# DiWu9/Union-Thesis-SLAM

Hardware: AMD Instinct MI355X
Metric: depth frames/sec (640x480 into 512^3 @ 2 cm dense TSDF; hash alongside) (higher is better)
Workload: dtype f64

## Files before the change

union-thesis-slam_amd/csrc/tsdf_common.hip:

```cpp
#include <unistd.h>

#include <algorithm>
#include <atomic>
#include <chrono>
#include <cmath>
#include <condition_variable>
#include <cstring>
#include <mutex>
#include <thread>
#include <vector>

#include "tsdf_host.h"

namespace tsdf {

static thread_local std::string g_err;

int set_error(int code, const char* fmt, ...) {
    char buf[1024];
    va_list ap;
    va_start(ap, fmt);
    vsnprintf(buf, sizeof(buf), fmt, ap);
    va_end(ap);
    g_err = buf;
// ... 404 lines not shown
        if (c0 < (size_t)n) {
            TSDF_HIP(hipMemcpyAsync((char*)st_depth[slot] + dbytes * c0, (const char*)hst_depth[slot] + dbytes * c0,
                                    dbytes * (n - c0), hipMemcpyHostToDevice, cstream));
            TSDF_HIP(hipMemcpyAsync((char*)st_color[slot] + cbytes * c0, (const char*)hst_color[slot] + cbytes * c0,
                                    cbytes * (n - c0), hipMemcpyHostToDevice, cstream));
        }
        TSDF_HIP(hipEventRecord(ev_copied[slot], cstream));
        TSDF_HIP(hipStreamWaitEvent(stream, ev_copied[slot], 0));
        d = (const char*)st_depth[slot];
        c = (const char*)st_color[slot];
    }
    const bool mask = (flags & TSDF_DEPTH_INVALID_65535) && dk == TSDF_DEPTH_U16_MM;
    if (mask && (dmask_px < npx || !dmask_set[n_sets - 1])) {
        TSDF_TRY(sync_all());
        for (int k = 0; k < kSets; ++k) {
            if (dmask_set[k]) TSDF_HIP(hipFree(dmask_set[k]));
            dmask_set[k] = nullptr;
        }
        for (int k = 0; k < n_sets; ++k)
            TSDF_HIP(hipMalloc(&dmask_set[k], sizeof(unsigned short) * npx * batch));
        dmask_px = npx;
    }
    use_set(cur_set);
    bt->n = n;
    const bool tex = texel_now && dk == TSDF_DEPTH_U16_MM && ck == TSDF_COLOR_RGB8;
    bt->texel = tex ? 1 : 0;
    for (int i = 0; i < n; ++i) {
        Frame* fr = &bt->f[i];
        const double* T = Tinv + 16 * (size_t)(first + i);
        for (int r = 0; r < 12; ++r) fr->T[r] = T[r];
        fr->fx = (double)(float)K[0];
        fr->fy = (double)(float)K[4];
        fr->cx = (double)(float)K[2];
        fr->cy = (double)(float)K[5];
        for (int j = 0; j < 4; ++j) {
            fr->Tf[j] = T[j] * fr->fx;
            fr->Tf[4 + j] = T[4 + j] * fr->fy;
        }
        {
            double wmax[3];
            for (int a = 0; a < 3; ++a) {
                const long long gmax = (a == 0 ? (long long)vol.off[0] + col_gx(vol, vol.nb[0] - 1) + kBrickEdge
                                               : (long long)vol.off[a] + vol.dims[a]);
                wmax[a] = fabs((double)vol.origin[a]) + vol.vs * (double)gmax + 1.0;
            }
            const PixelFixed pf = pixel_fixed(T, fr->fx, fr->fy, fr->cx, fr->cy, W, H, wmax);
            fr->Cx = pf.Cx;
            fr->Cy = pf.Cy;
            fr->mm = pf.mm;
            fr->whm1 = pf.whm1;
            fr->wmul = pf.wmul;
            fr->zmin_hi = pf.zmin_hi;
        }
        fr->ow = ow ? ow[first + i] : ow_default;
        fr->ow32 = (float)fr->ow;
        fr->H = H;
        fr->W = W;
        fr->depth_src = d + dbytes * i;
        fr->depth_mask = mask ? dmask + npx * i : nullptr;
        fr->depth = mask ? (const void*)fr->depth_mask : fr->depth_src;
        fr->color = c + cbytes * i;
        const bool direct = ck == TSDF_COLOR_RGB8 && rgb_direct &&
                            (!(flags & TSDF_DEVICE_PTRS) || (call_color_end && (const char*)fr->color + cbytes < call_color_end));
        if (tex) fr->rgbx = rgbx + 2 * npx * i;
        else fr->rgbx = direct ? nullptr : rgbx + npx * i;
        fr->pyr = pyr + (size_t)lay.total * i;

        frustum_planes(fr, T, W, H);
    }
    for (int L = 0; L <= kPyrLevels; ++L) {
        bt->pg.off[L] = lay.off[L];
        bt->pg.w[L] = lay.w[L];
        bt->pg.h[L] = lay.h[L];
    }
    return TSDF_OK;
}

int Base::stage_alloc(size_t dbytes, size_t cbytes) {
    if (st_depth_bytes >= dbytes * batch && st_color_bytes >= cbytes * batch) return TSDF_OK;
    TSDF_TRY(sync_all());
    for (int k = 0; k < kSlots; ++k) {
        if (st_depth[k]) TSDF_HIP(hipFree(st_depth[k]));
        if (st_color[k]) TSDF_HIP(hipFree(st_color[k]));
        if (hst_depth[k]) TSDF_HIP(hipHostFree(hst_depth[k]));
        if (hst_color[k]) TSDF_HIP(hipHostFree(hst_color[k]));
        st_depth[k] = st_color[k] = hst_depth[k] = hst_color[k] = nullptr;
    }
    st_depth_bytes = st_color_bytes = 0;
    for (int k = 0; k < kSlots; ++k) {
        TSDF_HIP(hipMalloc(&st_depth[k], dbytes * batch));
        TSDF_HIP(hipMalloc(&st_color[k], cbytes * batch + 64));
        TSDF_HIP(hipHostMalloc(&hst_depth[k], dbytes * batch, hipHostMallocDefault));
        TSDF_HIP(hipHostMalloc(&hst_color[k], cbytes * batch, hipHostMallocDefault));
    }
    st_depth_bytes = dbytes * batch;
    st_color_bytes = cbytes * batch;
    return TSDF_OK;
}

bool Base::defer_same(int dk, int ck, int H, int W, const double* K) const {
    return dfr.dk_in == dk && dfr.ck == ck && dfr.H == H && dfr.W == W && std::memcmp(dfr.K, K, sizeof(dfr.K)) == 0;
}

int Base::defer_push(const void* depth, int dk, const void* color, int ck, int H, int W,
                     const double* K, const double* T, double ow) {
    const size_t cbytes = frame_bytes_color(ck, H, W), npx = (size_t)H * W;
// ... 260 lines not shown
```

union-thesis-slam_amd/csrc/tsdf_device.h:

```cpp
#pragma once
#include <hip/hip_runtime.h>
#include <stdint.h>
#include <type_traits>

#include "tsdf_pixel.h"

namespace tsdf {

constexpr int kBrickEdge = 8;
constexpr int kBrickVox = 512;
constexpr int kWG = 256;
constexpr int kPyrLevels = 6;
constexpr int kStatSpread = 64;
constexpr unsigned long long kEmpty = ~0ull;
constexpr unsigned long long kTomb = ~0ull - 1ull;

enum Stat { ST_VOXELS = 0, ST_VISITED, ST_TOUCHED, ST_ALLOC, ST_PROBE, ST_LOOKUPS, ST_OVERFLOW,
            ST_PROBE_MAX, ST_BAD_ENTRY, ST_UNIQUE, kNStat };

struct Vol {
    int dims[3];
    int off[3];
    int xstride;
    int xodd;
    int sb[3];
    int nb[3];
    int shard, n_shards;
    int canon;
    float origin[3];
    double vs, trunc;
    double rtrunc;
    const double* rcp;
};

__host__ __device__ inline int col_gx(const Vol& v, int c) {
    return (c >> 1) * 2 * v.xstride + (c & 1) * v.xodd;
}

struct Frame {
    double T[12];
    double fx, fy, cx, cy;
    double ow;
    double Tf[8];
    double Cx, Cy;
    unsigned mm, whm1, wmul;
    int zmin_hi;
    float ow32;
    int H, W;
    const void* depth;
    const void* depth_src;
    unsigned short* depth_mask;
    const void* color;
    const unsigned* rgbx;
    const float* pyr;
    float planes[5][4];
    double eye[3];
};

struct PyrGeo {
    int off[kPyrLevels + 1];
    int w[kPyrLevels + 1];
    int h[kPyrLevels + 1];
};

#ifndef TSDF_MAX_BATCH
#define TSDF_MAX_BATCH 32
#endif
constexpr int kMaxBatch = TSDF_MAX_BATCH;
static_assert(kMaxBatch == 8 || kMaxBatch == 16 || kMaxBatch == 32, "frames per batch: 8, 16 or 32");
#ifndef TSDF_FULL_BATCH
#define TSDF_FULL_BATCH TSDF_MAX_BATCH
#endif
constexpr int kFullBatch = TSDF_FULL_BATCH < kMaxBatch ? TSDF_FULL_BATCH : kMaxBatch;
constexpr int kDoneWord = kMaxBatch + 8, kDoneWordC = kMaxBatch + 9, kCursorWord = kMaxBatch + 10;
constexpr int kCountWords = kMaxBatch + 16;
constexpr int kRcpTab = 4096;
constexpr int kRcpBig = 65536;

__device__ inline bool small_int(float w) {
    return w >= 0.0f && w < (float)(kRcpTab - kMaxBatch - 1) && w == truncf(w);
}
__device__ inline bool table_int(float w) {
    return w >= 0.0f && w < (float)(kRcpBig - kMaxBatch - 1) && w == truncf(w);
}
__device__ inline bool canon_color(float c) {
    return c >= 0.0f && c < 16777216.0f && c == truncf(c);
}
struct Batch {
    Frame f[kMaxBatch];
    PyrGeo pg;
    int n;
    int texel;
};

typedef unsigned long long ListEntry;

struct Pool {
    float* tsdf;
    float* weight;
// ... 20 lines not shown
struct Table {
    unsigned long long* keys;
    int* vals;
    unsigned long long* occ;
    int* free_list;
    ListEntry* overflow;
    PoolState* st;
    PoolReport* rb;
    long long capacity;
    long long shard_cap;
    long long max_blocks;
    const int* owned;
    int n_owned;
    int* ins_list;
    long long ins_cap;
    int overflow_cap;
    int int_bits;
};

template <bool POW2 = false>
__host__ __device__ inline long long ref_hash(long long x, long long y, long long z, long long n,
                                              int int_bits) {
    const unsigned long long P1 = 73856093ull, P2 = 19349669ull, P3 = 83492791ull;
    long long h;
    if (int_bits == 32) {
        const int a = (int)(unsigned)((unsigned long long)x * P1);
        const int b = (int)(unsigned)((unsigned long long)y * P2);
        const int c = (int)(unsigned)((unsigned long long)z * P3);
        h = (long long)(a ^ b ^ c);
    } else {
        h = (long long)(((unsigned long long)x * P1) ^ ((unsigned long long)y * P2) ^
                        ((unsigned long long)z * P3));
    }
    if (POW2 || (n & (n - 1)) == 0) return h & (n - 1);
    long long m = h % n;
    return m < 0 ? m + n : m;
}

template <bool POW2 = false>
__host__ __device__ inline int shard_of(long long home, int n_shards, long long cap) {
    if (POW2 || (cap & (cap - 1)) == 0) return (int)((home * n_shards) >> (63 - __builtin_clzll((unsigned long long)cap)));
    return (int)((home * n_shards) / cap);
}

__host__ __device__ inline unsigned long long pack_key(int bx, int by, int bz) {
    return (unsigned long long)bx | ((unsigned long long)by << 21) | ((unsigned long long)bz << 42);
}

__device__ inline int lane_id() { return threadIdx.x & 63; }

__device__ unsigned long long fcmp64_mask(double a, double b, int pred) __asm("llvm.amdgcn.fcmp.i64.f64");
__device__ unsigned long long fcmp32_mask(float a, float b, int pred) __asm("llvm.amdgcn.fcmp.i64.f32");
__device__ unsigned long long icmp32_mask(unsigned a, unsigned b, int pred) __asm("llvm.amdgcn.icmp.i64.i32");
constexpr int kCmpOGT = 2, kCmpOGE = 3, kCmpOLT = 4, kCmpUNE = 14, kCmpEQ = 32, kCmpNE = 33, kCmpULT = 36, kCmpSGT = 38;
__device__ inline bool lane_in(unsigned long long m) { return __builtin_amdgcn_inverse_ballot_w64(m); }
__device__ inline void sel_in_place(float& x, float y, unsigned long long m) {
    asm("v_cndmask_b32 %0, %0, %1, %2" : "+v"(x) : "v"(y), "s"(m));
}

template <typename T>
__device__ inline T coh_load(T* p) {
    return __hip_atomic_load(p, __ATOMIC_RELAXED, __HIP_MEMORY_SCOPE_AGENT);
}
template <typename T>
__device__ inline void coh_store(T* p, T v) {
    __hip_atomic_store(p, v, __ATOMIC_RELAXED, __HIP_MEMORY_SCOPE_AGENT);
}

__device__ inline int hash_find(const Table& t, int bx, int by, int bz, long long n_blocks) {
    const unsigned long long key = pack_key(bx, by, bz);
    long long s = ref_hash(bx, by, bz, t.capacity, t.int_bits);
    for (long long n = 0; n < t.capacity; ++n) {
        const unsigned long long k = coh_load(&t.keys[s]);
        if (k == key) {
            const int blk = coh_load(&t.vals[s]);
            return blk >= 0 && blk < n_blocks ? blk : -1;
        }
        if (k == kEmpty) return -1;
        if (++s == t.capacity) s = 0;
    }
    return -1;
}

__device__ inline double vox_world(float origin, double vs, int g) {
    return (double)(float)((double)origin + vs * (double)g);
}

struct BrickBox {
    double p0[3];
    float ext[3];
    float ctr[3];
    float rad;
};

__device__ inline BrickBox brick_box(const Vol& v, const double* eye, int bx, int by, int bz, int nx = 1,
                                     int ny = 1, int nz = 1) {
    const int bb[3] = {bx, by, bz}, nn[3] = {nx, ny, nz};
    BrickBox r;
#pragma unroll
    for (int a = 0; a < 3; ++a) {
        const int lo = bb[a] * kBrickEdge;
        const int hi = min(lo + nn[a] * kBrickEdge - 1, v.dims[a] - 1);
        const int glo = (a == 0) ? col_gx(v, bb[0]) : lo;
        const int ghi = (a == 0) ? col_gx(v, hi >> 3) + (hi & 7) : hi;
        r.p0[a] = (double)v.origin[a] + v.vs * (double)(glo + v.off[a]);
        r.ext[a] = (float)(v.vs * (double)(ghi - glo));
        r.ctr[a] = (float)(r.p0[a] + 0.5 * v.vs * (double)(ghi - glo) - eye[a]);
// ... 119 lines not shown
            if (ok == 2) {
                slot_out = target;
                probe = scanned + ((target - pos + t.capacity) % t.capacity);
                return coh_load(&t.vals[target]);
            }
            scanned += (target - pos + t.capacity) % t.capacity + 1;
            pos = target + 1;
            if (pos >= t.capacity) pos -= t.capacity;
            tomb = -1;
            continue;
        }
        pos += 64;
        if (pos >= t.capacity) pos -= t.capacity;
        scanned += 64;
    }
    return -1;
}


__device__ unsigned short buf_ld_u16(__amdgpu_buffer_rsrc_t r, int vindex, int voffset, int soffset,
                                     int aux) __asm("llvm.amdgcn.struct.ptr.buffer.load.i16");
__device__ unsigned buf_ld_u32(__amdgpu_buffer_rsrc_t r, int vindex, int voffset, int soffset,
                               int aux) __asm("llvm.amdgcn.struct.ptr.buffer.load.i32");
__device__ double buf_ld_f64(__amdgpu_buffer_rsrc_t r, int vindex, int voffset, int soffset,
                             int aux) __asm("llvm.amdgcn.struct.ptr.buffer.load.f64");
constexpr int kBufDword3 = 0x00020000;
typedef unsigned u32x2 __attribute__((ext_vector_type(2)));
__device__ u32x2 buf_ld_v2u32(__amdgpu_buffer_rsrc_t r, int vindex, int voffset, int soffset,
                              int aux) __asm("llvm.amdgcn.struct.ptr.buffer.load.v2i32");
struct FrameBufs {
    __amdgpu_buffer_rsrc_t depth, color;
};
template <int DK, int CK>
__device__ inline FrameBufs frame_bufs(const Frame& fr) {
    const int n = fr.W * fr.H;
    FrameBufs b;
    if (DK == 2) {
        static_assert(DK != 2 || CK == 0, "texels: RGB8 colour");
        b.depth = b.color = __builtin_amdgcn_make_buffer_rsrc((void*)fr.rgbx, 8, n, kBufDword3);
        return b;
    }
    b.depth = __builtin_amdgcn_make_buffer_rsrc((void*)fr.depth, DK == 0 ? 2 : 8, n, kBufDword3);
    if (CK == 0 && !fr.rgbx) b.color = __builtin_amdgcn_make_buffer_rsrc((void*)fr.color, 3, n, kBufDword3);
    else b.color = __builtin_amdgcn_make_buffer_rsrc((void*)(CK == 0 ? (const void*)fr.rgbx : fr.color), 4, n, kBufDword3);
    return b;
}
template <int DK>
__device__ inline unsigned depth_raw(const FrameBufs& fb, unsigned p) {
    return DK == 0 ? (unsigned)buf_ld_u16(fb.depth, (int)p, 0, 0, 0) : 0u;
}
template <int DK>
__device__ inline double depth_m(const FrameBufs& fb, unsigned p, unsigned raw) {
    if (DK != 1) {
        const double m = DK == 2 ? (double)(int)raw : (double)raw;
        return fma(m, 0.001, m * -2.0858186326137145e-20);
    }
    return buf_ld_f64(fb.depth, (int)p, 0, 0, 0);
}

__device__ inline double div_rn(double a, double b, double y) {
    const double q0 = a * y;
    const double r = fma(-q0, b, a);
    return fma(r, y, q0);
}

__device__ inline float div_rn32(float a, float b, float y) {
    const float q0 = a * y;
    const float r = fmaf(-q0, b, a);
    return fmaf(r, y, q0);
}

typedef float f2 __attribute__((ext_vector_type(2)));
__device__ inline f2 pk_fma(f2 a, f2 b, f2 c) { return __builtin_elementwise_fma(a, b, c); }
__device__ inline f2 rint2(f2 a) { return f2{rintf(a.x), rintf(a.y)}; }
__device__ inline f2 div_rn32x2(f2 a, f2 b, f2 y) {
    const f2 q0 = a * y;
    const f2 r = pk_fma(-q0, b, a);
    return pk_fma(r, y, q0);
}


__device__ inline int cvt_i32_sat(double x) {
    int r;
    asm("v_cvt_i32_f64 %0, %1" : "=v"(r) : "v"(x));
    return r;
}

typedef unsigned short u16x2 __attribute__((ext_vector_type(2)));
__device__ inline unsigned pk_min_u16(unsigned a, unsigned b) {
    return __builtin_bit_cast(unsigned, __builtin_elementwise_min(__builtin_bit_cast(u16x2, a), __builtin_bit_cast(u16x2, b)));
}
__device__ inline unsigned dot2_u16(unsigned a, unsigned b) {
    return __builtin_amdgcn_udot2(__builtin_bit_cast(u16x2, a), __builtin_bit_cast(u16x2, b), 0u, false);
}

__device__ inline double readlane_f64(double x, int l) {
    const unsigned long long u = __double_as_longlong(x);
    const unsigned lo = __builtin_amdgcn_readlane((unsigned)u, l);
    const unsigned hi = __builtin_amdgcn_readlane((unsigned)(u >> 32), l);
    return __longlong_as_double(((long long)hi << 32) | lo);
}


#ifdef TSDF_DIAG
__device__ unsigned long long g_ddiag[8];
#define TSDF_DDIAG(i) (lane_id() == 0 ? (void)atomicAdd(&g_ddiag[i], 1ull) : (void)0)
#else
#define TSDF_DDIAG(i) ((void)0)
#endif

template <int DK, int CK, int NZ>
__device__ __forceinline__ void project_part(double trunc, const Frame& fr, double px, double py,
                                             const double* pzs, double pz_l, int zoff, unsigned long long colm,
                                             int nz, unsigned (&cpx)[NZ], double (&diff)[NZ],
                                             unsigned long long (&okm)[NZ]) {
    constexpr int kPz = NZ < 8 ? NZ : 1;
    const double a2 = fma(fr.T[9], py, fr.T[8] * px);
    const double b0 = fma(fr.Tf[1], py, fma(fr.Tf[0], px, fr.Tf[3]));
    const double b1 = fma(fr.Tf[5], py, fma(fr.Tf[4], px, fr.Tf[7]));
    double zc[NZ];
    unsigned long long cand[NZ], slow[NZ], any_slow = 0;
    unsigned pix[NZ];
#pragma unroll
    for (int k = 0; k < NZ; ++k) {
        const double pz = NZ < 8 ? pzs[k % kPz] : readlane_f64(pz_l, k + zoff);
        zc[k] = fr.T[11] + fma(fr.T[10], pz, a2);
    }
    double rzs[NZ];
#pragma unroll
    for (int k = 0; k < NZ; ++k) rzs[k] = __builtin_amdgcn_rcp(zc[k]);
#pragma unroll
    for (int k = 0; k < NZ; ++k) {
        const double pz = NZ < 8 ? pzs[k % kPz] : readlane_f64(pz_l, k + zoff);
        const double z = zc[k], rz = rzs[k];
        const double tx = fma(fma(fr.Tf[2], pz, b0), rz, fr.Cx), ty = fma(fma(fr.Tf[6], pz, b1), rz, fr.Cy);
        const unsigned lx = (unsigned)__double_as_longlong(tx), ly = (unsigned)__double_as_longlong(ty);
        const unsigned P = __builtin_amdgcn_perm(ly, lx, 0x05040100u);
        const unsigned Q = __builtin_amdgcn_perm(ly, lx, 0x07060302u);
        const unsigned long long fine = icmp32_mask(pk_min_u16(P, fr.mm), fr.mm, kCmpEQ) &
                                        icmp32_mask((unsigned)(__double_as_longlong(z) >> 32), (unsigned)fr.zmin_hi, kCmpSGT);
        const unsigned long long col = k < nz ? colm : 0ull;
        cand[k] = col & fine & icmp32_mask(pk_min_u16(Q, fr.whm1), Q, kCmpEQ);
        pix[k] = lane_in(cand[k]) ? dot2_u16(Q, fr.wmul) : 0u;
        slow[k] = col & ~fine;
        any_slow |= slow[k];
    }
    TSDF_DDIAG(0);
    if (any_slow) {
        TSDF_DDIAG(3);
        const double a0 = fma(fr.T[1], py, fr.T[0] * px);
        const double a1 = fma(fr.T[5], py, fr.T[4] * px);
        const int W = fr.W, H = fr.H;
#pragma unroll
        for (int k = 0; k < NZ; ++k) {
            slow[k] &= fcmp64_mask(zc[k], 0.0, kCmpOGT);
            if (!slow[k]) continue;
            if (lane_in(slow[k])) {
                TSDF_DDIAG(2);
                const double pz = NZ < 8 ? pzs[k % kPz] : readlane_f64(pz_l, k + zoff);
                const double x = fr.T[3] + fma(fr.T[2], pz, a0);
                const double y = fr.T[7] + fma(fr.T[6], pz, a1);
                const int iu = cvt_i32_sat(rint((x * fr.fx) / zc[k] + fr.cx));
                const int iv = cvt_i32_sat(rint((y * fr.fy) / zc[k] + fr.cy));
                const bool inb = (unsigned)iu < (unsigned)W && (unsigned)iv < (unsigned)H;
                pix[k] = inb ? __umul24((unsigned)iv, (unsigned)W) + (unsigned)iu : ~0u;
            }
            cand[k] |= slow[k] & icmp32_mask(pix[k], ~0u, kCmpNE);
            pix[k] = lane_in(cand[k]) ? pix[k] : 0u;
        }
    }
    const FrameBufs fb = frame_bufs<DK, CK>(fr);
    unsigned draw[NZ];
#pragma unroll
    for (int k = 0; k < NZ; ++k) {
        if (DK == 2) {
            const u32x2 t = buf_ld_v2u32(fb.depth, (int)pix[k], 0, 0, 0);
            draw[k] = t.x;
            cpx[k] = t.y;
        } else {
            draw[k] = depth_raw<DK>(fb, pix[k]);
            cpx[k] = buf_ld_u32(fb.color, (int)pix[k], 0, 0, 0);
        }
    }
    __builtin_amdgcn_sched_barrier(0);
    double dep[NZ];
#pragma unroll
    for (int k = 0; k < NZ; ++k) dep[k] = depth_m<DK>(fb, pix[k], draw[k]);
#pragma unroll
    for (int k = 0; k < NZ; ++k) {
        diff[k] = dep[k] - zc[k];
        const unsigned long long dpos = DK == 2 ? ~0ull : DK == 0 ? icmp32_mask(draw[k], 0u, kCmpNE) : fcmp64_mask(dep[k], 0.0, kCmpOGT);
        okm[k] = cand[k] & dpos & fcmp64_mask(diff[k], -trunc, kCmpOGE);
    }
}

__device__ inline double dist_of(double trunc, double rtrunc, double diff) {
    return fmin(div_rn(diff, trunc, rtrunc), 1.0);
}

constexpr int kResFree = -1, kResFail = -3;

template <bool HASH, int DK, int CK, bool OW1, int NZ, bool CU = false>
__device__ inline void integrate_brick(const Vol& v, const Batch& bt, const Pool& pool,
                                       const Table& tab, ListEntry entry, int zoff,
                                       unsigned long long* s_stat, const double* s_rcp,
                                       unsigned& nupd, unsigned& nuniq, int* res = nullptr) {
    static_assert(!CU || (CK == 0 && OW1), "u32 colour registers: RGB8 frames, obs_weight 1");
    static_assert(NZ == 8 || NZ == 4, "z-parts of 8 or 4 steps");
    constexpr bool kHalfHash = HASH && NZ == 4;
    const int lane = lane_id();
    const int b = __builtin_amdgcn_readfirstlane((int)(entry & 0xFFFFFFFFull));
    const unsigned fmask = __builtin_amdgcn_readfirstlane((unsigned)(entry >> 32));
    const double trunc = v.trunc, rtrunc = v.rtrunc;
    const double* const rcp_hbm = v.rcp;
    const bool canon = CU || v.canon != 0;
    const int nb12 = v.nb[1] * v.nb[2];
    if (b >= v.nb[0] * nb12) {
        if (lane == 0) atomicAdd(&s_stat[ST_BAD_ENTRY], 1ull);
        return;
    }
    const int bx = b / nb12;
    const int rem = b - bx * nb12;
    const int by = rem / v.nb[2];
    const int bz = rem - by * v.nb[2];
    const int lx = bx * kBrickEdge + (lane >> 3);
    const int ly = by * kBrickEdge + (lane & 7);
    const unsigned long long colm = __ballot(lx < v.dims[0] && ly < v.dims[1]);
    const int nz = min(kBrickEdge, v.dims[2] - bz * kBrickEdge) - zoff;
    const double px = vox_world(v.origin[0], v.vs, v.off[0] + col_gx(v, bx) + (lane >> 3));
    const double py = vox_world(v.origin[1], v.vs, v.off[1] + ly);
    const double pz_l = vox_world(v.origin[2], v.vs, v.off[2] + bz * kBrickEdge + (lane & 7));
    constexpr int kPz = NZ < 8 ? NZ : 1;
    double pzs[kPz];
#pragma unroll
    for (int k = 0; k < kPz; ++k) {
        pzs[k] = readlane_f64(pz_l, k + zoff);
        if (NZ < 8) asm("" : "+v"(pzs[k]));
    }

    typename std::conditional<HASH, int, long long>::type blk = HASH ? -1 : b;
    bool is_new = false;
    bool upd = false;
    if constexpr (kHalfHash) {
        const int cur = __builtin_amdgcn_readfirstlane(res[b]);
        if (cur == kResFail) {
            if (zoff == 0 && lane == 0) {
                const unsigned long long o = atomicAdd((unsigned long long*)&tab.st->n_overflow, 1ull);
                if ((long long)o < tab.overflow_cap) tab.overflow[o] = entry;
                atomicAdd(&s_stat[ST_OVERFLOW], 1ull);
            }
            return;
        }
        if (cur < 0 || cur >= tab.max_blocks) {
            if (lane == 0) atomicAdd(&s_stat[ST_BAD_ENTRY], 1ull);
            return;
        }
        blk = cur;
    }
    float ws[NZ], ts[NZ], cs[NZ];
#pragma unroll
    for (int k = 0; k < NZ; ++k) {
        ws[k] = 0.0f;
        ts[k] = 1.0f;
        cs[k] = 0.0f;
    }
    constexpr int kH = NZ / 4;
    unsigned long long loaded[kH];
#pragma unroll
    for (int h = 0; h < kH; ++h) loaded[h] = 0;
    unsigned long long touched[NZ] = {};
    bool w_small = true;
    bool w_table = true;
    bool c_canon = true;
    bool fast_t = OW1 && s_rcp, table_t = false, fast_c = CK == 0 && fast_t;

#ifdef TSDF_DIAG
    int d_pairs = 0, d_valid = 0;
#endif
    for (unsigned fm = bt.n >= 32 ? fmask : fmask & ((1u << bt.n) - 1u); fm != 0; fm &= fm - 1u) {
        const Frame& fr = bt.f[__builtin_ctz(fm)];
#ifdef TSDF_DIAG
        ++d_pairs;
#endif
        unsigned cpx[NZ];
        double diff[NZ];
        unsigned long long okv[NZ];
        project_part<DK, CK, NZ>(trunc, fr, px, py, pzs, pz_l, zoff, colm, nz, cpx, diff, okv);
        unsigned long long need[kH];
#pragma unroll
        for (int h = 0; h < kH; ++h) need[h] = okv[4 * h] | okv[4 * h + 1] | okv[4 * h + 2] | okv[4 * h + 3];
        if ((need[0] | need[kH - 1]) == 0) continue;
        TSDF_DDIAG(1);
#ifdef TSDF_DIAG
        ++d_valid;
#endif

        upd = true;
        if (HASH && !kHalfHash && blk < 0) {
            if (HASH) {
                long long slot = 0, probe = 0;
                const unsigned long long key = pack_key(bx, by, bz);
                const long long home = ref_hash<kHalfHash>(bx, by, bz, tab.capacity, tab.int_bits);
                const int r = table_find_or_insert(tab, key, home, true, is_new, slot, probe);
                if (r < 0) {
                    if (lane == 0) {
                        const unsigned long long o = atomicAdd((unsigned long long*)&tab.st->n_overflow, 1ull);
                        if ((long long)o < tab.overflow_cap) tab.overflow[o] = entry;
                        atomicAdd(&s_stat[ST_OVERFLOW], 1ull);
                    }
                    return;
                }
                blk = r;
                if (is_new) {
#pragma unroll
                    for (int h = 0; h < kH; ++h) loaded[h] = ~0ull;
                }
                if (lane == 0) {
                    atomicAdd(&s_stat[ST_LOOKUPS], 1ull);
                    atomicAdd(&s_stat[ST_PROBE], (unsigned long long)probe);
                    atomicMax(&s_stat[ST_PROBE_MAX], (unsigned long long)probe);
                    if (is_new) atomicAdd(&s_stat[ST_ALLOC], 1ull);
                }
            } else {
                blk = b;
            }
        }
        unsigned long long ld[kH];
        unsigned long long any_ld = 0;
#pragma unroll
        for (int h = 0; h < kH; ++h) {
            ld[h] = need[h] & ~loaded[h];
            any_ld |= ld[h];
        }
        if (any_ld) {
            const size_t base = (size_t)blk * kBrickVox + (size_t)lane * kBrickEdge + zoff;
#pragma unroll
            for (int h = 0; h < kH; ++h) {
                if (!lane_in(ld[h])) continue;
                const float4 W = *(const float4*)(pool.weight + base + 4 * h);
                const float4 T = *(const float4*)(pool.tsdf + base + 4 * h);
                const float4 C = *(const float4*)(pool.color + base + 4 * h);
                ws[4 * h + 0] = W.x; ws[4 * h + 1] = W.y; ws[4 * h + 2] = W.z; ws[4 * h + 3] = W.w;
                if (canon) {
                    const float wm = fmaxf(fmaxf(W.x, W.y), fmaxf(W.z, W.w));
                    w_small = w_small && wm < (float)(kRcpTab - kMaxBatch - 1);
                    w_table = w_table && wm < (float)(kRcpBig - kMaxBatch - 1);
                } else {
                    w_small = w_small && small_int(W.x) && small_int(W.y) && small_int(W.z) && small_int(W.w);
                    w_table = w_table && table_int(W.x) && table_int(W.y) && table_int(W.z) && table_int(W.w);
                    c_canon = c_canon && canon_color(C.x) && canon_color(C.y) && canon_color(C.z) && canon_color(C.w);
                }
                ts[4 * h + 0] = T.x; ts[4 * h + 1] = T.y; ts[4 * h + 2] = T.z; ts[4 * h + 3] = T.w;
                if (CU) {
                    cs[4 * h + 0] = __uint_as_float((unsigned)C.x); cs[4 * h + 1] = __uint_as_float((unsigned)C.y);
                    cs[4 * h + 2] = __uint_as_float((unsigned)C.z); cs[4 * h + 3] = __uint_as_float((unsigned)C.w);
                } else {
                    cs[4 * h + 0] = C.x; cs[4 * h + 1] = C.y; cs[4 * h + 2] = C.z; cs[4 * h + 3] = C.w;
                }
            }
            fast_t = OW1 && s_rcp && __ballot(!w_small) == 0;
            table_t = OW1 && s_rcp && !fast_t && __ballot(!w_table) == 0;
            fast_c = CK == 0 && (fast_t || table_t) && __ballot(!c_canon) == 0;
        }
#pragma unroll
        for (int h = 0; h < kH; ++h) loaded[h] |= need[h];
#pragma unroll
        for (int k = 0; k < NZ; ++k) {
            const unsigned long long m = okv[k];
            touched[k] |= m;
            nupd += (unsigned)__popcll(m);
        }
        float wnv[NZ], cnv[NZ];
        if (!fast_c) TSDF_DDIAG(5);
        if (fast_c) {
            const __amdgpu_buffer_rsrc_t rt = __builtin_amdgcn_make_buffer_rsrc((void*)rcp_hbm, 0, kRcpBig * 8, kBufDword3);
            unsigned long long busy = 0;
#pragma unroll
            for (int k = 0; k < NZ; ++k)
                busy |= okv[k] & (fcmp64_mask(diff[k], trunc, kCmpOLT) | fcmp32_mask(ts[k], 1.0f, kCmpUNE));
            const bool free_space = busy == 0;
            if (free_space) TSDF_DDIAG(4);
            const auto pairs = [&](auto free_tag) {
            constexpr bool kFree = decltype(free_tag)::value;
#pragma unroll
            for (int k = 0; k < NZ; k += 2) {
                const f2 w2 = {ws[k], ws[k + 1]};
                const f2 a8 = pk_fma(w2, f2{8.0f, 8.0f}, f2{8.0f, 8.0f});
                const unsigned o0 = (unsigned)a8.x, o1 = (unsigned)a8.y;
                double y[2];
                if (fast_t) {
                    y[0] = *(const double*)((const char*)s_rcp + o0);
                    y[1] = *(const double*)((const char*)s_rcp + o1);
                } else {
                    y[0] = __longlong_as_double((long long)__builtin_amdgcn_raw_buffer_load_b64(rt, o0, 0, 0));
                    y[1] = __longlong_as_double((long long)__builtin_amdgcn_raw_buffer_load_b64(rt, o1, 0, 0));
                }
                const f2 wn2 = w2 + 1.0f;
                f2 r2;
                if constexpr (kFree) {
#pragma unroll
                    for (int j = 0; j < 2; ++j) r2[j] = (float)y[j];
                } else {
#pragma unroll
                    for (int j = 0; j < 2; ++j) {
                        const double num = (double)(w2[j] * ts[k + j]) + dist_of(trunc, rtrunc, diff[k + j]);
                        const float q = (float)div_rn(num, (double)wn2[j], y[j]);
                        sel_in_place(ts[k + j], q, okv[k + j]);
                        r2[j] = (float)y[j];
                    }
                }
                const unsigned c0 = CU ? __float_as_uint(cs[k]) : (unsigned)cs[k];
                const unsigned c1 = CU ? __float_as_uint(cs[k + 1]) : (unsigned)cs[k + 1];
                const f2 ob = {(float)((c0 >> 16) & 0xFFu), (float)((c1 >> 16) & 0xFFu)};
                const f2 nb = {(float)((cpx[k] >> 16) & 0xFFu), (float)((cpx[k + 1] >> 16) & 0xFFu)};
                const f2 qb = div_rn32x2(pk_fma(w2, ob, nb), wn2, r2);
                const f2 og = {(float)((c0 >> 8) & 0xFFu), (float)((c1 >> 8) & 0xFFu)};
                const f2 ng = {(float)((cpx[k] >> 8) & 0xFFu), (float)((cpx[k + 1] >> 8) & 0xFFu)};
                const f2 qg = div_rn32x2(pk_fma(w2, og, ng), wn2, r2);
                const f2 orr = {(float)(c0 & 0xFFu), (float)(c1 & 0xFFu)};
                const f2 nr = {(float)(cpx[k] & 0xFFu), (float)(cpx[k + 1] & 0xFFu)};
                const f2 qr = div_rn32x2(pk_fma(w2, orr, nr), wn2, r2);
                wnv[k] = wn2.x;
                wnv[k + 1] = wn2.y;
                if (CU) {
#pragma unroll
                    for (int j = 0; j < 2; ++j)
                        cnv[k + j] = __uint_as_float(__builtin_amdgcn_cvt_pk_u8_f32(
                            qb[j], 2, __builtin_amdgcn_cvt_pk_u8_f32(qg[j], 1, __builtin_amdgcn_cvt_pk_u8_f32(qr[j], 0, 0u))));
                } else {
                    const f2 rb = rint2(qb), rg = rint2(qg), rr = rint2(qr);
                    const f2 cn2 = pk_fma(rb, f2{65536.0f, 65536.0f}, pk_fma(rg, f2{256.0f, 256.0f}, rr));
                    cnv[k] = cn2.x;
                    cnv[k + 1] = cn2.y;
                }
            }
            };
            if (free_space) pairs(std::true_type{});
            else pairs(std::false_type{});
        } else {
#pragma unroll
            for (int k = 0; k < NZ; ++k) {
                const float w_old = ws[k];
                const float wn = OW1 ? w_old + 1.0f : (float)((double)w_old + fr.ow);
                const double dist = dist_of(trunc, rtrunc, diff[k]);
                const double num = (double)(w_old * ts[k]) + (OW1 ? dist : fr.ow * dist);
                float q;
                if (fast_t) q = (float)div_rn(num, (double)wn, s_rcp[(int)wn]);
                else if (table_t) q = (float)div_rn(num, (double)wn, rcp_hbm[(int)wn]);
                else q = (float)(num / (double)wn);
                wnv[k] = wn;
                float nb, ng, nr;
                if (CK == 0) {
                    nr = (float)(cpx[k] & 0xFFu);
                    ng = (float)((cpx[k] >> 8) & 0xFFu);
                    nb = (float)((cpx[k] >> 16) & 0xFFu);
                } else {
                    const float nc = __uint_as_float(cpx[k]);
                    nb = floorf(nc / 65536.0f);
                    ng = floorf((nc - nb * 65536.0f) / 256.0f);
                    nr = nc - nb * 65536.0f - ng * 256.0f;
                }
                const float co = CU ? (float)__float_as_uint(cs[k]) : cs[k];
                const float ob = floorf(co / 65536.0f);
                const float og = floorf((co - ob * 65536.0f) / 256.0f);
                const float orr = co - ob * 65536.0f - og * 256.0f;
                const float cb = fminf(255.0f, rintf((w_old * ob + (OW1 ? nb : fr.ow32 * nb)) / wn));
                const float cg = fminf(255.0f, rintf((w_old * og + (OW1 ? ng : fr.ow32 * ng)) / wn));
                const float cr = fminf(255.0f, rintf((w_old * orr + (OW1 ? nr : fr.ow32 * nr)) / wn));
                cnv[k] = CU ? __uint_as_float((unsigned)(cb * 65536.0f + cg * 256.0f + cr))
                            : cb * 65536.0f + cg * 256.0f + cr;
                ts[k] = lane_in(okv[k]) ? q : ts[k];
            }
        }
#pragma unroll
        for (int k = 0; k < NZ; ++k) {
            ws[k] = lane_in(okv[k]) ? wnv[k] : ws[k];
            cs[k] = lane_in(okv[k]) ? cnv[k] : cs[k];
        }
    }
#ifdef TSDF_DIAG
    if (!HASH && lane == 0) {
        atomicAdd(&s_stat[ST_PROBE], (unsigned long long)d_pairs);
        atomicAdd(&s_stat[ST_LOOKUPS], (unsigned long long)d_valid);
    }
#endif
    if constexpr (kHalfHash) {
        unsigned long long any = 0;
#pragma unroll
        for (int k = 0; k < NZ; ++k) any |= touched[k];
        if (any == 0) return;
    } else if (!upd) {
        return;
    }

#pragma unroll
    for (int k = 0; k < NZ; ++k) nuniq += (unsigned)__popcll(touched[k]);
    const size_t base = (size_t)blk * kBrickVox + (size_t)lane * kBrickEdge + zoff;
#pragma unroll
    for (int h = 0; h < kH; ++h) {
        if (!lane_in(loaded[h])) continue;
        *(float4*)(pool.weight + base + 4 * h) = make_float4(ws[4 * h], ws[4 * h + 1], ws[4 * h + 2], ws[4 * h + 3]);
        *(float4*)(pool.tsdf + base + 4 * h) = make_float4(ts[4 * h], ts[4 * h + 1], ts[4 * h + 2], ts[4 * h + 3]);
        if (CU)
            *(float4*)(pool.color + base + 4 * h) =
                make_float4((float)__float_as_uint(cs[4 * h]), (float)__float_as_uint(cs[4 * h + 1]),
                            (float)__float_as_uint(cs[4 * h + 2]), (float)__float_as_uint(cs[4 * h + 3]));
        else
            *(float4*)(pool.color + base + 4 * h) = make_float4(cs[4 * h], cs[4 * h + 1], cs[4 * h + 2], cs[4 * h + 3]);
    }
    if constexpr (HASH) {
        unsigned long long mine = 0;
#pragma unroll
        for (int k = 0; k < NZ; ++k) {
            if (lane == k) mine = touched[k];
        }
        if (lane < NZ) {
            unsigned long long* o = tab.occ + (size_t)blk * kBrickEdge + zoff + lane;
            if (is_new) coh_store(o, mine);
            else if (mine) atomicOr(o, mine);
        }
    }
    if (lane == 0) atomicAdd(&s_stat[ST_TOUCHED], 1ull);
}

__device__ inline void flush_stats(unsigned long long* s_stat, unsigned long long* stats) {
// ... 452 lines not shown
    if (t < n * n) {
        const int rr = t / n, cc = t - rr * n;
        const float m = fmaxf(fmaxf(src[2 * rr][2 * cc], src[2 * rr][2 * cc + 1]),
                              fmaxf(src[2 * rr + 1][2 * cc], src[2 * rr + 1][2 * cc + 1]));
        dst[rr][cc] = m;
        const int X = tx * n + cc, Y = ty * n + rr;
        if (X < pg.w[L] && Y < pg.h[L]) pyr[pg.off[L] + Y * pg.w[L] + X] = m;
    }
}

template <int DK = 0>
__device__ inline void prep_vec_tile(const Batch& bt, unsigned int* count, int tx, int ty, int tf,
                                     float (*sa)[33], float (*sb)[33]) {
    const Frame& fr = bt.f[tf];
    float* pyr = (float*)fr.pyr;
    const int t = threadIdx.x, r = t >> 4, c = t & 15;
    if (count && t < kCountWords && tx == 0 && ty == 0 && tf == 0) coh_store(count + t, 0u);
    const bool act = t < 512;
    const int x0 = tx * 64 + c * 4, y0 = ty * 64 + r * 2;
    float ma = 0.0f, mb = 0.0f;
    if (act && x0 < fr.W) {
#pragma unroll
        for (int dy = 0; dy < 2; ++dy) {
            const int y = y0 + dy;
            if (y >= fr.H) continue;
            const size_t p = (size_t)y * fr.W + x0;
            uint2 dd = make_uint2(0u, 0u);
            if (DK == 1) {
                const double2 d0 = *(const double2*)((const double*)fr.depth_src + p);
                const double2 d1 = *(const double2*)((const double*)fr.depth_src + p + 2);
                ma = fmaxf(ma, fmaxf((float)d0.x, (float)d0.y));
                mb = fmaxf(mb, fmaxf((float)d1.x, (float)d1.y));
            } else {
                dd = *(const uint2*)((const unsigned short*)fr.depth_src + p);
                if (fr.depth_mask) {
                    unsigned lo0 = dd.x & 0xFFFFu, hi0 = dd.x >> 16, lo1 = dd.y & 0xFFFFu, hi1 = dd.y >> 16;
                    lo0 = lo0 == 65535u ? 0u : lo0;
                    hi0 = hi0 == 65535u ? 0u : hi0;
                    lo1 = lo1 == 65535u ? 0u : lo1;
                    hi1 = hi1 == 65535u ? 0u : hi1;
                    dd = make_uint2(lo0 | (hi0 << 16), lo1 | (hi1 << 16));
                    *(uint2*)(fr.depth_mask + p) = dd;
                }
                ma = fmaxf(ma, fmaxf((float)(dd.x & 0xFFFFu) * 1e-3f, (float)(dd.x >> 16) * 1e-3f));
                mb = fmaxf(mb, fmaxf((float)(dd.y & 0xFFFFu) * 1e-3f, (float)(dd.y >> 16) * 1e-3f));
            }
            if (fr.rgbx) {
                const unsigned* q = (const unsigned*)((const unsigned char*)fr.color + 3 * p);
                const unsigned a = q[0], b = q[1], cc = q[2];
                const uint4 c4 = make_uint4(a & 0xFFFFFFu, (a >> 24) | ((b & 0xFFFFu) << 8),
                                            (b >> 16) | ((cc & 0xFFu) << 16), cc >> 8);
                if (DK == 2) {
                    uint4* t = (uint4*)((uint2*)fr.rgbx + p);
                    const auto dw = [](unsigned d) { return d ? d : TSDF_TEXEL_INVALID; };
                    t[0] = make_uint4(dw(dd.x & 0xFFFFu), c4.x, dw(dd.x >> 16), c4.y);
                    t[1] = make_uint4(dw(dd.y & 0xFFFFu), c4.z, dw(dd.y >> 16), c4.w);
                } else {
                    *(uint4*)((unsigned*)fr.rgbx + p) = c4;
                }
            }
        }
    }
    const PyrGeo& pg = bt.pg;
    const auto put = [&](int L, int X, int Y, float m) {
        if (X < pg.w[L] && Y < pg.h[L]) pyr[pg.off[L] + Y * pg.w[L] + X] = m;
    };
    if (act) {
        const int X = x0 >> 1, Y = y0 >> 1;
        put(1, X, Y, ma);
        put(1, X + 1, Y, mb);
    }
    float m2 = fmaxf(ma, mb);
    m2 = fmaxf(m2, __shfl_down(m2, 16));
    if (act && (r & 1) == 0) put(2, tx * 16 + c, ty * 16 + (r >> 1), m2);
    float m3 = fmaxf(m2, __shfl_down(m2, 1));
    m3 = fmaxf(m3, __shfl_down(m3, 32));
    if (act && (r & 3) == 0 && (c & 1) == 0) {
        put(3, tx * 8 + (c >> 1), ty * 8 + (r >> 2), m3);
        sa[r >> 2][c >> 1] = m3;
    }
    __syncthreads();
    if (t < 64) {
        const int lx = t & 7, ly = t >> 3;
        float m = sa[ly][lx];
        m = fmaxf(m, __shfl_down(m, 1));
        m = fmaxf(m, __shfl_down(m, 8));
        if ((lx & 1) == 0 && (ly & 1) == 0) put(4, tx * 4 + (lx >> 1), ty * 4 + (ly >> 1), m);
        m = fmaxf(m, __shfl_down(m, 2));
        m = fmaxf(m, __shfl_down(m, 16));
        if ((lx & 3) == 0 && (ly & 3) == 0) put(5, tx * 2 + (lx >> 2), ty * 2 + (ly >> 2), m);
        m = fmaxf(m, __shfl_down(m, 4));
        m = fmaxf(m, __shfl_down(m, 32));
        if (t == 0) put(6, tx, ty, m);
    }
    (void)sb;
}

template <int DK = 0>
__global__ __launch_bounds__(512) void k_prep_vec(Batch bt, unsigned int* count) {
    __shared__ float sa[32][33];
    __shared__ float sb[32][33];
    prep_vec_tile<DK>(bt, count, blockIdx.x, blockIdx.y, blockIdx.z, sa, sb);
}

template <int DK, int CK>
__global__ __launch_bounds__(1024) void k_prep(Batch bt, unsigned int* count) {
    __shared__ float sa[32][33];
// ... 252 lines not shown
```

union-thesis-slam_amd/csrc/tsdf_host.h:

```cpp
#pragma once
#include <hip/hip_runtime.h>

#include <cstdarg>
#include <cstdlib>
#include <cstdio>
#include <string>
#include <utility>
#include <vector>

#include "tsdf_device.h"
#include "tsdf_hip.h"

#ifndef TSDF_CULL_WAVES_DEFAULT
#define TSDF_CULL_WAVES_DEFAULT 2
#endif

namespace tsdf {

int set_error(int code, const char* fmt, ...);

#define TSDF_HIP(expr)                                                                        \
    do {                                                                                      \
        hipError_t e_ = (expr);                                                               \
        if (e_ != hipSuccess)                                                                 \
// ... 3 lines not shown
    } while (0)

#define TSDF_TRY(expr)            \
    do {                          \
        int r_ = (expr);          \
        if (r_ != TSDF_OK) return r_; \
    } while (0)

inline size_t frame_bytes_depth(int dk, int H, int W) { return (size_t)H * W * (dk == TSDF_DEPTH_U16_MM ? 2 : 8); }
inline size_t frame_bytes_color(int ck, int H, int W) { return (size_t)H * W * (ck == TSDF_COLOR_RGB8 ? 3 : 4); }

struct PyrLayout {
    int off[kPyrLevels + 1];
    int w[kPyrLevels + 1];
    int h[kPyrLevels + 1];
    int total;
};
PyrLayout pyr_layout(int H, int W);

struct Profiler {
    bool on = false;
    std::vector<std::pair<hipEvent_t, hipEvent_t>> pending;
    std::vector<hipEvent_t> spare;
    double ms = 0.0;
    long long launches = 0;
    int begin(hipStream_t s, hipEvent_t* e0);
    int end(hipStream_t s, hipEvent_t e0);
    int collect();
    void release();
};

constexpr int kSets = 3;
constexpr int kSlots = 4;

struct IcpCtx;
void icp_ctx_free(IcpCtx* c);

struct Base {
    int device = 0;
    hipStream_t stream = nullptr;
    Vol vol{};
    Pool pool{};
    long long n_bricks = 0;
    int batch = kMaxBatch;
    int set_batch(int want);
    int defer_frames = 8;
    int dma_grain = 2;
    bool rgb_direct = true;
    int texel_mode = -1;
    bool texel_now = false;
    static constexpr long long kTexelMinBricksDense = 3ll << 14, kTexelMinBricksHash = 3ll << 15;
    bool texel_for(int dk, long long owned_bricks, long long min_bricks) const {
        if (dk != TSDF_DEPTH_U16_MM) return false;
        if (!(vol.trunc < TSDF_TEXEL_MAX_TRUNC)) return false;
        return texel_mode >= 0 ? texel_mode != 0 : owned_bricks >= min_bricks;
    }
    bool defer_mm = true;
    int mm_backoff = 0;
    static constexpr int kMmBackoff = 4;
    const char* call_color_end = nullptr;
    float* pyr = nullptr;
    unsigned* rgbx = nullptr;
    int pyr_H = 0, pyr_W = 0;
    ListEntry* list = nullptr;
    unsigned int* count = nullptr;
    float* pyr_set[kSets] = {};
    unsigned* rgbx_set[kSets] = {};
    ListEntry* list_set[kSets] = {};
    unsigned int* count_set[kSets] = {};
    unsigned short* dmask_set[kSets] = {};
    int n_sets = 1;
    int n_cu = 256;
    PyrLayout lay{};
    unsigned long long* stats = nullptr;
    double* rcp = nullptr;
    long long frames = 0;
    Profiler prof;
    hipStream_t cstream = nullptr;
    hipEvent_t ev_copied[kSlots] = {};
    hipEvent_t ev_free[kSlots] = {};
    void* st_depth[kSlots] = {};
    void* st_color[kSlots] = {};
    size_t st_depth_bytes = 0, st_color_bytes = 0;
    unsigned short* dmask = nullptr;
    size_t dmask_px = 0;
    void* hst_depth[kSlots] = {};
    void* hst_color[kSlots] = {};

    struct Deferred {
        int n = 0, H = 0, W = 0, dk = 0, ck = 0, slot = -1;
        int dk_in = 0;
        int copied = 0;
        double K[9];
        double T[16 * kMaxBatch];
        double ow[kMaxBatch];
    } dfr;
    int defer_next = 0;
    int prestaged = -1;
    int pre_copied = 0;
    bool defer_same(int dk, int ck, int H, int W, const double* K) const;
    int defer_push(const void* depth, int dk, const void* color, int ck, int H, int W,
                   const double* K, const double* T, double ow);
    static constexpr int kDeferFlush = 1;
    int stage_alloc(size_t dbytes, size_t cbytes);
    bool stage_fits(int dk, int ck, int H, int W) const {
        return st_depth_bytes >= frame_bytes_depth(dk, H, W) * batch &&
               st_color_bytes >= frame_bytes_color(ck, H, W) * batch;
// ... 111 lines not shown
```

union-thesis-slam_amd/csrc/tsdf_pixel.h:

```cpp
#ifndef TSDF_PIXEL_H
#define TSDF_PIXEL_H
#include <limits.h>
#include <math.h>
#include <string.h>

static inline double frame_margin(int W, int H, double cx, double cy) {
    const double span = (double)(W > H ? W : H) + fmax(fabs(cx), fabs(cy));
    return fmax(1e-4, 1e-7 * span);
}

static inline void fold_rows(const double* T, double fx, double fy, const double wmax[3], double out[2]) {
    for (int r = 0; r < 2; ++r) {
        const double* t = T + 4 * r;
        out[r] = (r == 0 ? fx : fy) *
                 (fabs(t[0]) * wmax[0] + fabs(t[1]) * wmax[1] + fabs(t[2]) * wmax[2] + fabs(t[3]));
    }
}

static inline double fold_bound(const double* T, double fx, double fy, const double wmax[3], double margin) {
    double b[2];
    fold_rows(T, fx, fy, wmax, b);
    return 4.0 * (8.0 * 0x1p-53 * fmax(b[0], b[1])) / margin;
}

// ... 2 lines not shown
typedef struct {
    double Cx, Cy;
    unsigned mm;
    unsigned whm1;
    unsigned wmul;
    int zmin_hi;
    int mx, my;
    double zmin;
} PixelFixed;

static inline int pixel_axis(double c, double margin, double* C) {
    const double C0 = (c + 0.5) + TSDF_PIXEL_BIAS;
    const double err = fabs(((C0 - TSDF_PIXEL_BIAS) - 0.5) - c);
    double m = ceil((margin + 0x1p-17 + err) * 65536.0);
    while (m * 0x1p-16 - 0x1p-17 - err < margin) m += 1.0;
    *C = C0 + m * 0x1p-16;
    return m < 32768.0 ? (int)m : -1;
}

static inline PixelFixed pixel_fixed(const double* T, double fx, double fy, double cx, double cy, int W,
                                     int H, const double wmax[3]) {
    PixelFixed p;
    memset(&p, 0, sizeof p);
    p.zmin_hi = INT_MAX;
    p.zmin = INFINITY;
    int finite = isfinite(fx) && isfinite(fy) && isfinite(cx) && isfinite(cy);
    for (int r = 0; r < 12; ++r) finite = finite && isfinite(T[r]);
    for (int j = 0; j < 4; ++j) finite = finite && isfinite(T[j] * fx) && isfinite(T[4 + j] * fy);
    if (!finite || W < 1 || H < 1 || W > 16384 || H > 16384) return p;
    const double margin = frame_margin(W, H, cx, cy);
    double b[2];
    fold_rows(T, fx, fy, wmax, b);
    const double denx = 65536.0 - (double)W - fabs(cx) - 2.0, deny = 65536.0 - (double)H - fabs(cy) - 2.0;
    if (!(denx >= 1.0) || !(deny >= 1.0)) return p;
    const double zmin = fmax(fold_bound(T, fx, fy, wmax, margin), fmax(b[0] / denx, b[1] / deny));
    double Cx, Cy;
    const int mx = pixel_axis(cx, margin, &Cx), my = pixel_axis(cy, margin, &Cy);
    if (mx < 0 || my < 0 || !isfinite(zmin) || !(zmin < 1e300)) return p;
    long long bits;
    memcpy(&bits, &zmin, sizeof bits);
    p.zmin_hi = (int)(bits >> 32) + 1;
    p.zmin = zmin;
    p.Cx = Cx;
    p.Cy = Cy;
    p.mx = mx;
    p.my = my;
    p.mm = ((unsigned)(2 * my) << 16) | (unsigned)(2 * mx);
    p.whm1 = ((unsigned)(H - 1) << 16) | (unsigned)(W - 1);
    p.wmul = ((unsigned)W << 16) | 1u;
    return p;
}

#define TSDF_TEXEL_INVALID 0x80000000u
#define TSDF_TEXEL_MAX_TRUNC 1.0e6
static inline double texel_depth_m(int raw) {
    const double m = (double)raw;
    return fma(m, 0.001, m * -2.0858186326137145e-20);
}

#endif
```

Measured before the change: 26890.

## Encode texel depth as f64 high-word key to skip free-space voxels early

Texel depth words now store the high 32 bits of (depth + trunc) plus a bias instead of raw millimetres. Projection compares each voxel's camera z high word against this key with integer compares, so out-of-band voxels are classified without decoding depth. When no voxel in the wave lies near the surface, it skips the f64 distance computation and uses a constant distance of 1. Depth is reconstructed from the key only when needed. This adds range limits on trunc and relies on conservative high-word bounds, which risks misclassifying edge cases.

```diff
diff --git a/union-thesis-slam_amd/csrc/tsdf_common.hip b/union-thesis-slam_amd/csrc/tsdf_common.hip
--- a/union-thesis-slam_amd/csrc/tsdf_common.hip
+++ b/union-thesis-slam_amd/csrc/tsdf_common.hip
@@ -480,6 +480,9 @@
             fr->wmul = pf.wmul;
             fr->zmin_hi = pf.zmin_hi;
         }
+        fr->kt = vol.trunc;
+        fr->c2 = tex ? depth_key_c2(vol.trunc) : 0.0;
+        fr->t1000 = 1000.0 * vol.trunc;
         fr->ow = ow ? ow[first + i] : ow_default;
         fr->ow32 = (float)fr->ow;
         fr->H = H;
diff --git a/union-thesis-slam_amd/csrc/tsdf_device.h b/union-thesis-slam_amd/csrc/tsdf_device.h
--- a/union-thesis-slam_amd/csrc/tsdf_device.h
+++ b/union-thesis-slam_amd/csrc/tsdf_device.h
@@ -45,6 +45,7 @@
     double Cx, Cy;
     unsigned mm, whm1, wmul;
     int zmin_hi;
+    double kt, c2, t1000;
     float ow32;
     int H, W;
     const void* depth;
@@ -171,7 +172,8 @@
 __device__ unsigned long long fcmp64_mask(double a, double b, int pred) __asm("llvm.amdgcn.fcmp.i64.f64");
 __device__ unsigned long long fcmp32_mask(float a, float b, int pred) __asm("llvm.amdgcn.fcmp.i64.f32");
 __device__ unsigned long long icmp32_mask(unsigned a, unsigned b, int pred) __asm("llvm.amdgcn.icmp.i64.i32");
-constexpr int kCmpOGT = 2, kCmpOGE = 3, kCmpOLT = 4, kCmpUNE = 14, kCmpEQ = 32, kCmpNE = 33, kCmpULT = 36, kCmpSGT = 38;
+constexpr int kCmpOGT = 2, kCmpOGE = 3, kCmpOLT = 4, kCmpUNE = 14, kCmpEQ = 32, kCmpNE = 33, kCmpULT = 36, kCmpSGT = 38, kCmpSGE = 39,
+              kCmpSLE = 41;
 __device__ inline bool lane_in(unsigned long long m) { return __builtin_amdgcn_inverse_ballot_w64(m); }
 __device__ inline void sel_in_place(float& x, float y, unsigned long long m) {
     asm("v_cndmask_b32 %0, %0, %1, %2" : "+v"(x) : "v"(y), "s"(m));
@@ -397,7 +399,7 @@
 template <int DK>
 __device__ inline double depth_m(const FrameBufs& fb, unsigned p, unsigned raw) {
     if (DK != 1) {
-        const double m = DK == 2 ? (double)(int)raw : (double)raw;
+        const double m = (double)raw;
         return fma(m, 0.001, m * -2.0858186326137145e-20);
     }
     return buf_ld_f64(fb.depth, (int)p, 0, 0, 0);
@@ -455,7 +457,7 @@
 #endif
 
 template <int DK, int CK, int NZ>
-__device__ __forceinline__ void project_part(double trunc, const Frame& fr, double px, double py,
+__device__ __forceinline__ bool project_part(double trunc, const Frame& fr, double px, double py,
                                              const double* pzs, double pz_l, int zoff, unsigned long long colm,
                                              int nz, unsigned (&cpx)[NZ], double (&diff)[NZ],
                                              unsigned long long (&okm)[NZ]) {
@@ -515,6 +517,7 @@
         }
     }
     const FrameBufs fb = frame_bufs<DK, CK>(fr);
+    const double c2 = DK == 2 ? fr.c2 : 0.0;
     unsigned draw[NZ];
 #pragma unroll
     for (int k = 0; k < NZ; ++k) {
@@ -528,15 +531,33 @@
         }
     }
     __builtin_amdgcn_sched_barrier(0);
+    if constexpr (DK == 2) {
+        unsigned long long geom = 0;
+#pragma unroll
+        for (int k = 0; k < NZ; ++k) {
+            okm[k] = cand[k] & icmp32_mask((unsigned)(__double_as_longlong(zc[k]) >> 32), draw[k], kCmpSLE);
+            geom |= okm[k] & icmp32_mask((unsigned)(__double_as_longlong(zc[k] + c2) >> 32), draw[k], kCmpSGE);
+        }
+        if (geom == 0) return false;
+        const double t1000 = fr.t1000;
+#pragma unroll
+        for (int k = 0; k < NZ; ++k) {
+            diff[k] = depth_key_depth(draw[k], t1000) - zc[k];
+            okm[k] = cand[k] & fcmp64_mask(diff[k], -trunc, kCmpOGE);
+            __builtin_amdgcn_sched_barrier(0);
+        }
+        return true;
+    }
     double dep[NZ];
 #pragma unroll
     for (int k = 0; k < NZ; ++k) dep[k] = depth_m<DK>(fb, pix[k], draw[k]);
 #pragma unroll
     for (int k = 0; k < NZ; ++k) {
         diff[k] = dep[k] - zc[k];
-        const unsigned long long dpos = DK == 2 ? ~0ull : DK == 0 ? icmp32_mask(draw[k], 0u, kCmpNE) : fcmp64_mask(dep[k], 0.0, kCmpOGT);
+        const unsigned long long dpos = DK == 0 ? icmp32_mask(draw[k], 0u, kCmpNE) : fcmp64_mask(dep[k], 0.0, kCmpOGT);
         okm[k] = cand[k] & dpos & fcmp64_mask(diff[k], -trunc, kCmpOGE);
     }
+    return true;
 }
 
 __device__ inline double dist_of(double trunc, double rtrunc, double diff) {
@@ -630,7 +651,7 @@
         unsigned cpx[NZ];
         double diff[NZ];
         unsigned long long okv[NZ];
-        project_part<DK, CK, NZ>(trunc, fr, px, py, pzs, pz_l, zoff, colm, nz, cpx, diff, okv);
+        const bool has_diff = project_part<DK, CK, NZ>(trunc, fr, px, py, pzs, pz_l, zoff, colm, nz, cpx, diff, okv);
         unsigned long long need[kH];
 #pragma unroll
         for (int h = 0; h < kH; ++h) need[h] = okv[4 * h] | okv[4 * h + 1] | okv[4 * h + 2] | okv[4 * h + 3];
@@ -719,14 +740,14 @@
         if (!fast_c) TSDF_DDIAG(5);
         if (fast_c) {
             const __amdgpu_buffer_rsrc_t rt = __builtin_amdgcn_make_buffer_rsrc((void*)rcp_hbm, 0, kRcpBig * 8, kBufDword3);
-            unsigned long long busy = 0;
+            unsigned long long busy = DK == 2 && has_diff ? ~0ull : 0ull;
 #pragma unroll
             for (int k = 0; k < NZ; ++k)
-                busy |= okv[k] & (fcmp64_mask(diff[k], trunc, kCmpOLT) | fcmp32_mask(ts[k], 1.0f, kCmpUNE));
+                busy |= okv[k] & ((DK == 2 ? 0ull : fcmp64_mask(diff[k], trunc, kCmpOLT)) | fcmp32_mask(ts[k], 1.0f, kCmpUNE));
             const bool free_space = busy == 0;
             if (free_space) TSDF_DDIAG(4);
-            const auto pairs = [&](auto free_tag) {
-            constexpr bool kFree = decltype(free_tag)::value;
+            const auto pairs = [&](auto free_tag, auto dist1_tag) {
+            constexpr bool kFree = decltype(free_tag)::value, kDist1 = decltype(dist1_tag)::value;
 #pragma unroll
             for (int k = 0; k < NZ; k += 2) {
                 const f2 w2 = {ws[k], ws[k + 1]};
@@ -748,7 +769,7 @@
                 } else {
 #pragma unroll
                     for (int j = 0; j < 2; ++j) {
-                        const double num = (double)(w2[j] * ts[k + j]) + dist_of(trunc, rtrunc, diff[k + j]);
+                        const double num = (double)(w2[j] * ts[k + j]) + (kDist1 ? 1.0 : dist_of(trunc, rtrunc, diff[k + j]));
                         const float q = (float)div_rn(num, (double)wn2[j], y[j]);
                         sel_in_place(ts[k + j], q, okv[k + j]);
                         r2[j] = (float)y[j];
@@ -780,14 +801,16 @@
                 }
             }
             };
-            if (free_space) pairs(std::true_type{});
-            else pairs(std::false_type{});
+            if (free_space) pairs(std::true_type{}, std::false_type{});
+            else if (DK != 2 || has_diff) pairs(std::false_type{}, std::false_type{});
+            else pairs(std::false_type{}, std::true_type{});
         } else {
+            const auto exact = [&](auto dist1_tag) {
 #pragma unroll
             for (int k = 0; k < NZ; ++k) {
                 const float w_old = ws[k];
                 const float wn = OW1 ? w_old + 1.0f : (float)((double)w_old + fr.ow);
-                const double dist = dist_of(trunc, rtrunc, diff[k]);
+                const double dist = decltype(dist1_tag)::value ? 1.0 : dist_of(trunc, rtrunc, diff[k]);
                 const double num = (double)(w_old * ts[k]) + (OW1 ? dist : fr.ow * dist);
                 float q;
                 if (fast_t) q = (float)div_rn(num, (double)wn, s_rcp[(int)wn]);
@@ -816,6 +839,9 @@
                             : cb * 65536.0f + cg * 256.0f + cr;
                 ts[k] = lane_in(okv[k]) ? q : ts[k];
             }
+            };
+            if (DK != 2 || has_diff) exact(std::false_type{});
+            else exact(std::true_type{});
         }
 #pragma unroll
         for (int k = 0; k < NZ; ++k) {
@@ -1374,7 +1400,8 @@
                                             (b >> 16) | ((cc & 0xFFu) << 16), cc >> 8);
                 if (DK == 2) {
                     uint4* t = (uint4*)((uint2*)fr.rgbx + p);
-                    const auto dw = [](unsigned d) { return d ? d : TSDF_TEXEL_INVALID; };
+                    const double kt = fr.kt;
+                    const auto dw = [kt](unsigned d) { return depth_key(d, kt); };
                     t[0] = make_uint4(dw(dd.x & 0xFFFFu), c4.x, dw(dd.x >> 16), c4.y);
                     t[1] = make_uint4(dw(dd.y & 0xFFFFu), c4.z, dw(dd.y >> 16), c4.w);
                 } else {
diff --git a/union-thesis-slam_amd/csrc/tsdf_host.h b/union-thesis-slam_amd/csrc/tsdf_host.h
--- a/union-thesis-slam_amd/csrc/tsdf_host.h
+++ b/union-thesis-slam_amd/csrc/tsdf_host.h
@@ -79,7 +79,7 @@
     static constexpr long long kTexelMinBricksDense = 3ll << 14, kTexelMinBricksHash = 3ll << 15;
     bool texel_for(int dk, long long owned_bricks, long long min_bricks) const {
         if (dk != TSDF_DEPTH_U16_MM) return false;
-        if (!(vol.trunc < TSDF_TEXEL_MAX_TRUNC)) return false;
+        if (!depth_key_trunc_ok(vol.trunc)) return false;
         return texel_mode >= 0 ? texel_mode != 0 : owned_bricks >= min_bricks;
     }
     bool defer_mm = true;
diff --git a/union-thesis-slam_amd/csrc/tsdf_pixel.h b/union-thesis-slam_amd/csrc/tsdf_pixel.h
--- a/union-thesis-slam_amd/csrc/tsdf_pixel.h
+++ b/union-thesis-slam_amd/csrc/tsdf_pixel.h
@@ -78,10 +78,40 @@
 }
 
 #define TSDF_TEXEL_INVALID 0x80000000u
-#define TSDF_TEXEL_MAX_TRUNC 1.0e6
-static inline double texel_depth_m(int raw) {
+#define TSDF_TEXEL_MAX_TRUNC 256.0
+#define TSDF_TEXEL_MIN_TRUNC 0x1p-20
+#ifdef __HIPCC__
+#define TSDF_HD __host__ __device__
+#else
+#define TSDF_HD
+#endif
+static inline TSDF_HD double texel_depth_m(int raw) {
     const double m = (double)raw;
     return fma(m, 0.001, m * -2.0858186326137145e-20);
 }
 
+static inline TSDF_HD int f64_hi(double x) {
+    long long b;
+    memcpy(&b, &x, sizeof b);
+    return (int)(b >> 32);
+}
+static inline double depth_key_eps(double t) { return ldexp(6.0, ilogb(65.535 + t) - 20); }
+static inline double depth_key_c2(double t) { return 2.0 * t + depth_key_eps(t); }
+static inline int depth_key_trunc_ok(double t) { return t >= TSDF_TEXEL_MIN_TRUNC && t < TSDF_TEXEL_MAX_TRUNC; }
+static inline TSDF_HD unsigned depth_key(unsigned m, double t) {
+    return m ? (unsigned)f64_hi(texel_depth_m((int)m) + t) + 2u : TSDF_TEXEL_INVALID;
+}
+static inline TSDF_HD int depth_key_sup(double z, unsigned key) { return f64_hi(z) <= (int)key; }
+static inline TSDF_HD int depth_key_near(double z, double c2, unsigned key) { return f64_hi(z + c2) >= (int)key; }
+static inline TSDF_HD double depth_key_mm(unsigned key, double t1000) {
+    const long long b = (long long)(unsigned long long)(key - 2u) << 32;
+    double val;
+    memcpy(&val, &b, sizeof val);
+    return rint(fma(val, 1000.0, -t1000));
+}
+static inline TSDF_HD double depth_key_depth(unsigned key, double t1000) {
+    const double m = depth_key_mm(key, t1000);
+    return fma(m, 0.001, m * -2.0858186326137145e-20);
+}
+
 #endif
```

Result: no change. 26870 (median of 2 runs) (-0.1%).
